# HaoruXue/spline-trajectory-optimization

Measured on AMD Instinct MI355X. Metric: min-curvature QP solves/sec (N=2000 waypoints), higher is better.
Workload: dtype f64

## Files before the change

### spline_trajectory_optimization_amd/csrc/rl_host.hpp

```cpp
#pragma once

#include "../../include/rl_mincurv.h"

#include <hip/hip_runtime.h>

#include <mutex>
#include <string>
#include <utility>
#include <vector>

namespace {

thread_local std::string g_err;

int fail(int code, const std::string& msg) {
  g_err = msg;
  return code;
}

#define RL_HIP(expr)                                                                      \
  do {                                                                                    \
    hipError_t _e = (expr);                                                               \
    if (_e != hipSuccess) {                                                               \
      return fail(RL_ERR_HIP, std::string(#expr) + ": " + hipGetErrorString(_e));         \
    }                                                                                     \
  } while (0)
#define RL_TRY(expr) do { if (int _rc = (expr)) return _rc; } while (0)

template <typename T>
struct DevBuf {
  T* p = nullptr;
  size_t n = 0;
  hipError_t alloc(size_t count) {
    release();
    n = count;
    if (count == 0) return hipSuccess;
    return hipMalloc(reinterpret_cast<void**>(&p), count * sizeof(T));
  }
  void release() {
    if (p) (void)hipFree(p);
    p = nullptr;
    n = 0;
  }
  ~DevBuf() { release(); }
  DevBuf() = default;
  DevBuf(const DevBuf&) = delete;
  DevBuf& operator=(const DevBuf&) = delete;
};

}

struct rl_ctx {
  int device = 0;
  hipStream_t stream = nullptr;
  hipEvent_t ev0 = nullptr, ev1 = nullptr;
  int max_lds = 65536;
  int num_cu = 0;
  bool force_global_v1 = false;
  int arith = RL_ARITH_REFERENCE;
  bool arith_explicit = false;
  int np_raise_at_start = 0;
  int qss_kernel = -1, qss_df_waves = 4, qss_df_bail_at = 0;
  int tables_search = RL_SEARCH_WINDOWED, tables_rings_global = 0;
  int frenet_search = 1;
  void* arena = nullptr;
  size_t arena_cap = 0;
  hipEvent_t arena_ev = nullptr;
  hipStream_t arena_stream = nullptr;
  bool arena_busy = false;
  static constexpr int kMaxGroups = 8;
  hipStream_t aux_stream[kMaxGroups - 1] = {};
  hipEvent_t ev_fork = nullptr, ev_join[kMaxGroups - 1] = {};
  hipStream_t poll_stream = nullptr;
  hipEvent_t ev_chunk[kMaxGroups] = {}, ev_poll[2] = {nullptr, nullptr};
  double* poll_host = nullptr;
  size_t poll_cap = 0;
  bool mt_hes_sweep = false;
  bool mt_kkt4 = true;
  bool mt_unfused = false;
  int mt_groups = 3;
  struct PoolBlock { void* p; size_t cap; bool used; };
  std::vector<PoolBlock> pool;
};

namespace {
hipError_t grant_dyn_lds(const rl_ctx* ctx, const void* fn, size_t bytes) {
  static std::mutex mu;
  static std::vector<std::pair<std::pair<int, const void*>, size_t>> granted;
  std::lock_guard<std::mutex> lock(mu);
  const std::pair<int, const void*> key(ctx->device, fn);
  for (auto& e : granted)
    if (e.first == key) {
      if (e.second >= bytes) return hipSuccess;
      const hipError_t r = hipFuncSetAttribute(fn, hipFuncAttributeMaxDynamicSharedMemorySize, (int)bytes);
      if (r == hipSuccess) e.second = bytes;
      return r;
    }
  const hipError_t r = hipFuncSetAttribute(fn, hipFuncAttributeMaxDynamicSharedMemorySize, (int)bytes);
  if (r == hipSuccess) granted.emplace_back(key, bytes);
  return r;
}

template <typename... P, typename... A>
int launch(const rl_ctx* ctx, hipStream_t stream, void (*kernel)(P...), dim3 grid, dim3 block, size_t lds_bytes, A&&... args) {
  if (lds_bytes > 0) RL_HIP(grant_dyn_lds(ctx, reinterpret_cast<const void*>(kernel), lds_bytes));
  hipLaunchKernelGGL(kernel, grid, block, lds_bytes, stream, static_cast<P>(std::forward<A>(args))...);
  RL_HIP(hipGetLastError());
  return RL_OK;
}
template <typename... P, typename... A>
int launch(const rl_ctx* ctx, void (*kernel)(P...), dim3 grid, dim3 block, size_t lds_bytes, A&&... args) {
  return launch(ctx, ctx->stream, kernel, grid, block, lds_bytes, std::forward<A>(args)...);
}

// ... 170 lines not shown
```

### spline_trajectory_optimization_amd/csrc/rl_mincurv.hip

```cpp
#include "rl_host.hpp"

#include <algorithm>
#include <cmath>
#include <cstdio>
#include <cstdlib>
#include <cstring>
#include <type_traits>

#include "rl_kernels.hpp"
#include "rl_sweep.hpp"
#include "rl_qss_df.hpp"
#include "rl_global.hpp"
#include "rl_global2.hpp"
#include "rl_global_xy.hpp"
#include "rl_dtrack.hpp"
#include "rl_mintime.hpp"
#include "rl_bicycle.hpp"
#include "rl_region.hpp"
#include "rl_tables.hpp"
#include "rl_pose_tables.hpp"
#include "rl_spline_fit.hpp"
#include "rl_frenet.hpp"

namespace {
// ... 264 lines not shown
    delete c;
    return fail(RL_ERR_HIP, "hipEventCreate failed");
  }
  *out = c;
  return RL_OK;
}

void rl_ctx_destroy(rl_ctx* ctx) {
  if (!ctx) return;
  if (ctx->arena) (void)hipFree(ctx->arena);
  if (ctx->arena_ev) (void)hipEventDestroy(ctx->arena_ev);
  for (auto& blk : ctx->pool)
    if (blk.p) (void)hipFree(blk.p);
  for (int g = 0; g < rl_ctx::kMaxGroups - 1; ++g) {
    if (ctx->aux_stream[g]) (void)hipStreamDestroy(ctx->aux_stream[g]);
    if (ctx->ev_join[g]) (void)hipEventDestroy(ctx->ev_join[g]);
  }
  if (ctx->ev_fork) (void)hipEventDestroy(ctx->ev_fork);
  if (ctx->poll_stream) (void)hipStreamDestroy(ctx->poll_stream);
  for (auto& e : ctx->ev_chunk) if (e) (void)hipEventDestroy(e);
  for (auto& e : ctx->ev_poll) if (e) (void)hipEventDestroy(e);
  if (ctx->poll_host) (void)hipHostFree(ctx->poll_host);
  if (ctx->ev0) (void)hipEventDestroy(ctx->ev0);
  if (ctx->ev1) (void)hipEventDestroy(ctx->ev1);
  delete ctx;
}

int rl_ctx_set_stream(rl_ctx* ctx, void* hip_stream) {
  if (!ctx) return fail(RL_ERR_ARG, "ctx is null");
  ctx->stream = reinterpret_cast<hipStream_t>(hip_stream);
  return RL_OK;
}

int rl_ctx_set_arith(rl_ctx* ctx, int arith) {
  if (!ctx) return fail(RL_ERR_ARG, "ctx is null");
  if (arith == RL_ARITH_DEFAULT) { ctx->arith = RL_ARITH_REFERENCE; ctx->arith_explicit = false; return RL_OK; }
  if (arith != RL_ARITH_FAST && arith != RL_ARITH_REFERENCE && arith != RL_ARITH_BRANCH)
    return fail(RL_ERR_ARG, "arith must be RL_ARITH_DEFAULT, RL_ARITH_FAST, RL_ARITH_REFERENCE or RL_ARITH_BRANCH");
  ctx->arith = arith;
  ctx->arith_explicit = true;
  return RL_OK;
}

int rl_ctx_get_arith(const rl_ctx* ctx) { return ctx ? (ctx->arith_explicit ? ctx->arith : RL_ARITH_DEFAULT) : RL_ERR_ARG; }

int rl_ctx_set_option(rl_ctx* ctx, const char* name, int value) {
  if (!ctx || !name) return fail(RL_ERR_ARG, "null argument");
  const std::string k(name);
  if (k == "qss_kernel") { if (value < -1 || value > 1) return fail(RL_ERR_ARG, "qss_kernel: -1 (auto), 0 (list order), 1 (dataflow)"); ctx->qss_kernel = value; }
  else if (k == "qss_df_waves") { if (value != 1 && value != 2 && value != 4) return fail(RL_ERR_ARG, "qss_df_waves: 1, 2 or 4"); ctx->qss_df_waves = value; }
  else if (k == "qss_df_bail_at") { if (value < 0) return fail(RL_ERR_ARG, "qss_df_bail_at >= 0"); ctx->qss_df_bail_at = value; }
  else if (k == "tables_search") { if (value < RL_SEARCH_BRUTE || value > RL_SEARCH_WINDOWED) return fail(RL_ERR_ARG, "tables_search: RL_SEARCH_BRUTE, _CULLED or _WINDOWED"); ctx->tables_search = value; }
  else if (k == "tables_rings") { if (value != 0 && value != 1) return fail(RL_ERR_ARG, "tables_rings: 0 (LDS where they fit) or 1 (arena)"); ctx->tables_rings_global = value; }
  else if (k == "frenet_search") { if (value != 0 && value != 1) return fail(RL_ERR_ARG, "frenet_search: 0 (table bound for every point) or 1 (from the previous point's piece)"); ctx->frenet_search = value; }
  else return fail(RL_ERR_ARG, "unknown option '" + k + "'");
  return RL_OK;
}

int rl_ctx_set_numpy_raise(rl_ctx* ctx, int on) {
  if (!ctx) return fail(RL_ERR_ARG, "ctx is null");
  ctx->np_raise_at_start = on ? 1 : 0;
  return RL_OK;
}

int rl_debug_cr_heading(rl_ctx* ctx, const double* dx, const double* dy, int n, double* out) {
  if (!ctx || !dx || !dy || !out || n <= 0) return fail(RL_ERR_ARG, "bad argument");
  Staging sg(ctx);
  const double* ddx = sg.in(dx, n);
  const double* ddy = sg.in(dy, n);
  double* dout = sg.out(out, (size_t)5 * n);
  sg.run([&] { return launch(ctx, rl::k_debug_cr_heading, dim3((n + 255) / 256), dim3(256), 0, ddx, ddy, n, dout); });
  return sg.finish();
}

int rl_ctx_synchronize(rl_ctx* ctx) {
  if (!ctx) return fail(RL_ERR_ARG, "ctx is null");
  RL_HIP(hipStreamSynchronize(ctx->stream));
  return RL_OK;
}

int rl_spline_eval(rl_ctx* ctx, const double* t, int nt, const double* cx, const double* cy, int k,
                   const double* u, int N, int der_max, double* out) {
  if (!ctx || !u || !out) return fail(RL_ERR_ARG, "null argument");
  if (int rc = check_spline(t, nt, cx, cy, k)) return rc;
  if (N <= 0 || der_max < 0 || der_max > 2) return fail(RL_ERR_ARG, "bad N / der_max");
  const int n = nt - k - 1;
  Staging sg(ctx);
  const double *dt = sg.in(t, nt), *dcx = sg.in(cx, n), *dcy = sg.in(cy, n), *du = sg.in(u, N);
  double* dout = sg.out(out, (size_t)2 * (der_max + 1) * N);
  sg.run([&] {
    return by_degree(k, [&](auto kc) {
      return launch(ctx, rl::k_spline_eval<RL_DEGREE(kc)>, dim3((N + 255) / 256), dim3(256), 0, dt, nt, dcx, dcy, du, N, der_max, dout);
    });
  });
  return sg.finish();
}

int rl_sample_along(rl_ctx* ctx, const double* t, int nt, const double* cx, const double* cy, int k,
                    double length, const double* u, int N, double* points) {
  if (!ctx || !u || !points) return fail(RL_ERR_ARG, "null argument");
  if (int rc = check_spline(t, nt, cx, cy, k)) return rc;
  if (N <= 0) return fail(RL_ERR_ARG, "bad N");
  const int n = nt - k - 1;
  Staging sg(ctx);
  const double *dt = sg.in(t, nt), *dcx = sg.in(cx, n), *dcy = sg.in(cy, n), *du = sg.in(u, N);
  double* dpts = sg.out(points, (size_t)N * RL_NCOL);
// ... 170 lines not shown
    }
    if (widest > rl::kJointRowsPerThread * 256)
      return fail(RL_ERR_UNSUPPORTED, "sliding-window variant: a window spans more than 768 samples");
  }
  int arith = ctx->arith;
  if (!ctx->arith_explicit && arith == RL_ARITH_REFERENCE && (k != 5 || (g_dbg_instances > 0 && !from))) arith = RL_ARITH_FAST;
  const bool lite = arith == RL_ARITH_BRANCH;
  const bool strict = arith == RL_ARITH_REFERENCE || lite;
  if (strict) {
    if (joint && lite) return fail(RL_ERR_UNSUPPORTED, "the branch arithmetic (rl_ctx_set_arith) covers run_min_curvature_qp; the sliding-window driver exists in the fast and in the reference-order arithmetic");
    RL_HIP(hipSetDevice(ctx->device));
    if (int rc = ensure_strict_tables(ctx, trk)) return rc;
  }
  rl::SweepArgs a;
  std::memset(&a, 0, sizeof(a));
  a.tr = trk->dev();
  a.B = B;
  a.form = form;
  a.in = in_dev;
  Bounds bd;
  if (int rc = resolve_bounds(trk, form, in_dev, bd)) return rc;
  a.ringL = bd.ringL; a.ringR = bd.ringR; a.nL = bd.nL; a.nR = bd.nR;
  a.max_iter = max_iter;
  for (int j = 0; j < max_iter && !i_start_rows; ++j) a.i_start[j] = i_start[j];
  a.ctrl0 = ctrl0; a.i_start_rows = i_start_rows;
  a.search = search;
  a.max_dist = 100.0;
#ifdef RL_ABLATION
  if (const char* dbg = getenv("RL_DEBUG_FLAGS")) a.debug = atoi(dbg);
#endif
#ifdef RL_STAMPS
  const bool dbg_ok = true;
#else
  const bool dbg_ok = !strict;
#endif
  if (g_dbg_instances > 0 && (joint || k == 5) && dbg_ok && !from) {
    const int ninst = std::min(g_dbg_instances, B);
    size_t need = joint ? (size_t)max_iter * (size_t)(i_max - i_min) * (48 + 9 * rl::kJointRowsPerThread * 256 + 2 * n)
                        : (size_t)ninst * max_iter * 2 * (size_t)(i_max - i_min) * (rl::kSweepDumpHead + 2 * n);
#ifdef RL_STAMPS
    need = std::max(need, (size_t)B * 4 * 16);
#endif
    a.dbg_instances = ninst;
    if (g_dbg_len < need) {
      if (g_dbg_buf) (void)hipFree(g_dbg_buf);
      RL_HIP(hipMalloc(reinterpret_cast<void**>(&g_dbg_buf), need * sizeof(double)));
      g_dbg_len = need;
    }
    RL_HIP(hipMemsetAsync(g_dbg_buf, 0, need * sizeof(double), ctx->stream));
    a.dbg = g_dbg_buf;
  }
  a.out_ctrl = out_ctrl; a.out_xy = out_xy; a.out_points = out_points;
  a.n_success = n_success; a.status = status;
  RL_HIP(hipSetDevice(ctx->device));
  SweepPlan p = plan_sweep(ctx, n, N, a.nL, a.nR, B, joint, strict);
  if (p.lds_bytes > (size_t)ctx->max_lds) return fail(RL_ERR_UNSUPPORTED, "problem does not fit LDS");
  if (p.residency == rl::Residency::CrossingsLds && (joint || k != 5 || a.dbg || from)) {
    p.residency = rl::Residency::Global;
    p.lds_bytes = rl::sweep_lds_layout(n, N, a.nL, a.nR, rl::Residency::Global, joint).total * sizeof(double);
    p.gscratch_doubles += (size_t)2 * ((N + 1) & ~1);
  }
  if (p.gscratch_doubles) {
    const size_t need = p.gscratch_doubles * (size_t)B;
    if (trk->gscratch.n < need) RL_HIP(trk->gscratch.alloc(need));
    a.gscratch = trk->gscratch.p;
    a.gscratch_stride = p.gscratch_doubles;
  }
  if (strict && !lite) {
    const size_t per = (size_t)2 * ((n + 1) & ~1) + (size_t)2 * ((N + 15) / 16) + (size_t)2 * N;
    const size_t flags = ((size_t)B + 1) / 2;
    if (trk->aux.n < per * (size_t)B + flags) RL_HIP(trk->aux.alloc(per * (size_t)B + flags));
    a.aux = trk->aux.p;
    a.aux_stride = per;
    a.np_raise_at_start = ctx->np_raise_at_start;
    a.raise_flag = reinterpret_cast<int*>(trk->aux.p + per * (size_t)B);
    RL_HIP(hipMemsetAsync(a.raise_flag, 0, (size_t)B * sizeof(int), ctx->stream));
  }
  if (stats) {
    stats->lds_bytes = (int)p.lds_bytes;
    stats->block_threads = p.block;
    stats->rings_in_lds = p.residency == rl::Residency::Lds ? 1 : (p.residency == rl::Residency::CrossingsLds ? 2 : 0);
    stats->reserved[0] = arith;
  }
  if (plan_out) *plan_out = p;
  if (from) return launch_sweep_from(ctx, k, p, a, strict, lite);
  return launch_sweep(ctx, k, p, a, joint, strict, lite);
}

int rl_mincurv_solve_batch_dev(rl_ctx* ctx, const rl_track* trk, int bounds_form, const double* in,
                               int B, const int* i_start, int max_iter, int search,
                               double* out_ctrl, double* out_xy, int* n_success, int* status,
                               rl_stats* stats) {
  if (!out_xy) return fail(RL_ERR_ARG, "out_xy is null");
  return solve_batch_common(ctx, trk, bounds_form, in, B, i_start, max_iter, search, out_ctrl, out_xy,
                            nullptr, n_success, status, stats, nullptr);
}

int rl_mincurv_solve_batch_host(rl_ctx* ctx, const rl_track* trk, int bounds_form, const double* in,
                                int B, const int* i_start, int max_iter, int search,
                                double* out_ctrl, double* out_xy, int* n_success, int* status,
                                rl_stats* stats) {
  if (!ctx || !trk || !out_ctrl || !out_xy) return fail(RL_ERR_ARG, "null argument");
  if (B <= 0) return fail(RL_ERR_ARG, "B <= 0");
  const int n = trk->n, N = trk->N;
  const int cols = bounds_cols(bounds_form);
  if (cols && !in) return fail(RL_ERR_ARG, "bounds input is null");
// ... 1088 lines not shown
```

### spline_trajectory_optimization_amd/csrc/rl_sweep.hpp

```cpp
#pragma once
#include "rl_kernels.hpp"

namespace rl {

constexpr int kJointRowsPerThread = 3;

struct SweepArgs {
  TrackDev tr;
  int B;
  int form;
  const double* in;
  const double2* ringL;
  const double2* ringR;
  int nL, nR;
  int max_iter;
  int i_start[32];
  int search;
  double max_dist;
  double* out_ctrl;
  double* out_xy;
  double* out_points;
  int* n_success;
  int* status;
  double* gscratch;
  size_t gscratch_stride;
  double* dbg;
  int dbg_instances;
  int debug;
  int np_raise_at_start;
  double* aux;
  size_t aux_stride;
  int* n_raised;
  int* raise_flag;
  const double* ctrl0;
  const int* i_start_rows;
};

#ifdef RL_STAMPS
#define RL_STAMP(var) do { __builtin_amdgcn_sched_barrier(0); asm volatile("s_memtime %0\n\ts_waitcnt lgkmcnt(0)" : "=s"(var) :: "memory"); __builtin_amdgcn_sched_barrier(0); } while (0)
#define RL_STAMP_ADD(slot, t1, t0) st_acc[slot] += (t1) - (t0)
#define RL_STRICT_COUNTS st_cnt
#define RL_FSTAMP(slot) do { RL_STAMP(sf1); st_fine[slot] += sf1 - sf0; sf0 = sf1; } while (0)
#else
#define RL_STAMP(var) do { } while (0)
#define RL_STAMP_ADD(slot, t1, t0) do { } while (0)
#define RL_STRICT_COUNTS nullptr
#define RL_FSTAMP(slot) do { } while (0)
#endif

#ifdef RL_ABLATION
#define RL_ABLATE(a, bit) (((a).debug & (bit)) != 0)
#else
#define RL_ABLATE(a, bit) false
#endif

enum class Residency { Lds, Global, CrossingsLds };

struct SweepLds {
  int cpad, nLp, nRp, ncL, ncR;
  size_t off_cx, off_cy, off_red, off_sL, off_sR, off_rL, off_rR, off_cL, off_cR, off_pL, off_pR, off_hint, off_joint, off_stage,
         off_c12, off_terms, total;
};
constexpr int kSweepWaves = 4;
constexpr int kSweepThreads = kWave * kSweepWaves;
constexpr int kTermChunk = 256;
constexpr int kTermStride = kTermChunk + 2;
constexpr int kC12Doubles = 4 * (2 * kMaxK) + 8;
constexpr int kRedCoordMax = 194;

__host__ __device__ inline SweepLds sweep_lds_layout(int n, int N, int nL, int nR, Residency residency,
                                                     bool joint = false, bool strict = false) {
  const bool rings_in_lds = residency == Residency::Lds, sigma_in_lds = residency != Residency::Global;
  SweepLds L;
  L.cpad = (n + 1) & ~1;
  L.nLp = nL; L.nRp = nR;
  L.ncL = (nL + kChunk - 1) / kChunk;
  L.ncR = (nR + kChunk - 1) / kChunk;
  size_t o = 0;
  L.off_cx = o; o += L.cpad;
  L.off_cy = o; o += L.cpad;
  L.off_red = o; o += 8 * 24 + 4;
  L.off_cL = o; o += (size_t)((3 * L.ncL + 1) & ~1);
  L.off_cR = o; o += (size_t)((3 * L.ncR + 1) & ~1);
  L.off_pL = o; o += (size_t)((L.ncL + 1) & ~1);
  L.off_pR = o; o += (size_t)((L.ncR + 1) & ~1);
  L.off_joint = o; o += joint ? 128 + (size_t)((N + 15) / 16) * 2 : 0;
  L.off_hint = o; o += (size_t)(((size_t)2 * ((N + 3) & ~3) * sizeof(unsigned short) + 15) / 16) * 2;
  L.off_c12 = o; o += strict ? (joint ? (size_t)4 * L.cpad : kC12Doubles) : 0;
// ... 167 lines not shown
        for (int q = 0; q < nc; ++q) {
          int dq = q - cc;
          if (dq < 0) dq = -dq;
          if (nc - dq < dq) dq = nc - dq;
          if (dq <= kNear) continue;
          const double ex = circ[3 * q] - mx, ey = circ[3 * q + 1] - my;
          gap = fmin(gap, sqrt(ex * ex + ey * ey) - r - circ[3 * q + 2]);
        }
        (left ? sepL : sepR)[cc] = gap * (1.0 - 1e-9) - 1e-9;
      }
      if (wave == 0) {
        double m = 0.0;
        for (int c = lane; c < L.ncL + L.ncR; c += kWave) {
          const double* o = c < L.ncL ? circL + 3 * c : circR + 3 * (c - L.ncL);
          const double v = fmax(fabs(o[0]), fabs(o[1])) + o[2];
          m = v <= 0x1p+1000 ? fmax(m, v) : INFINITY;
        }
        m = wave_max_bfly(m);
        if (lane == 0) red[kRedCoordMax] = m;
      }
      __syncthreads();
    }
  }

  double* jq = smem + L.off_joint;
  unsigned char* outside = reinterpret_cast<unsigned char*>(jq + 128);
  int* n_outside = reinterpret_cast<int*>(jq + 127);
  auto note_outside = [&](int i, double px, double py, double ndx, double ndy, double sl, double sr) {
    const double Lx = px + sl * ndx, Ly = py + sl * ndy;
    const double Rx = px + sr * (-ndx), Ry = py + sr * (-ndy);
    const bool out = fmin(Lx, Rx) > px || fmax(Lx, Rx) < px || fmin(Ly, Ry) > py || fmax(Ly, Ry) < py;
    const int was = outside[i];
    if ((int)out != was) { outside[i] = out ? 1 : 0; atomicAdd(n_outside, out ? 1 : -1); }
  };
  auto note_outside_pts = [&](int i, double px, double py, double2 Lp, double2 Rp) {
    const bool out = fmin(Lp.x, Rp.x) > px || fmax(Lp.x, Rp.x) < px || fmin(Lp.y, Rp.y) > py || fmax(Lp.y, Rp.y) < py;
    const int was = outside[i];
    if ((int)out != was) { outside[i] = out ? 1 : 0; atomicAdd(n_outside, out ? 1 : -1); }
  };
  if (JOINT) {
    for (int i = tid; i < N; i += BLOCK) outside[i] = 0;
    if (tid == 0) *n_outside = 0;
    __syncthreads();
  }

#ifdef RL_STAMPS
  unsigned long long st_cnt[4] = {0, 0, 0, 0};
  unsigned long long st_fine[8] = {0, 0, 0, 0, 0, 0, 0, 0}, sf0 = 0, sf1 = 0;
#endif
  unsigned char* degen = (RAISE && a.aux) ? reinterpret_cast<unsigned char*>(a.aux + (size_t)b * a.aux_stride + 2 * L.cpad) : nullptr;
  int* n_degen = reinterpret_cast<int*>(red + 190);
  bool flag_mode = false;
  bool saw_degenerate = false;
  auto refresh = [&](int i0, int i1, int j0, int j1, int mode, int l_first = -1) {
    const int m0 = i1 - i0, m1 = j1 - j0, m = m0 + m1;
    const double* cmax = red + kRedCoordMax;
    if constexpr (STRICT) {
      int delta = 0;
      auto point = [&](int i, double& px, double& py, cr::Heading& hd, bool flags, auto&& in_heading) {
#pragma clang fp contract(off)
        const int l = tr.ell[i];
        double t0[K + 1], t1[K + 1];
        load_rows<K + 1>(t0, Ds + (size_t)SR::D0 * N, N, i);
        load_rows<K + 1>(t1, Ds + (size_t)SR::D1 * N, N, i);
        __builtin_amdgcn_sched_barrier(0);
        px = seq_dot_v<K + 1>(cx + (l - K), t0);
        py = seq_dot_v<K + 1>(cy + (l - K), t0);
        const double tx = seq_dot_v<K + 1>(cx + (l - K), t1);
        const double ty = seq_dot_v<K + 1>(cy + (l - K), t1);

        if constexpr (LITE && RL_LITE_NORMAL) {
          double nx, ny, inv_s2;
          scaled_normal(tx, ty, 1.0, nx, ny, inv_s2);
          hd.cl = nx; hd.sl = ny; hd.cr = -nx; hd.sr = -ny; hd.yaw = 0.0;
          return;
        }
        if (flags) {
          const double d2x = seq_dot<K + 1>(cx + (l - K), Ds + (size_t)SR::D2 * N, N, i);
          const double d2y = seq_dot<K + 1>(cy + (l - K), Ds + (size_t)SR::D2 * N, N, i);
          const double s2 = tx * tx + ty * ty;
          const double cross = fabs(tx * d2y - ty * d2x);
          const bool plainly_regular = cross >= 0x1p-200 && cross <= 0x1p+200 && s2 >= 0x1p-100 && s2 <= 0x1p+100;
          int now = 0;
          if (!__all(plainly_regular)) {
            const double den = sqrt(s2 * s2 * s2);
            const double curvature = cross / den;
            now = (den == 0.0 || !(curvature > 0.0) || !isfinite(curvature)) ? 1 : 0;
          }
          if constexpr (RAISE) { delta += now - (int)degen[i]; degen[i] = (unsigned char)now; }
          else if (now) saw_degenerate = true;
        }
#ifdef RL_STAMPS
        unsigned long long sh0, sh1;
        RL_STAMP(sh0);
#endif
        const bool sure = cr::heading_fast(tx, ty, hd, cr::kAtanTab, nullptr, in_heading);
        if (__any(!sure)) { if (!sure) hd = cr::heading(tx, ty); }
#ifdef RL_STAMPS
        RL_STAMP(sh1); st_fine[5] += sh1 - sh0; if (__any(!sure)) st_fine[6] += 1;
#endif
      };
      if (mode == 2) {
        const int nwt = (m + kWave - 1) / kWave;
        for (int wt = wave; wt < nwt; wt += NW) {
          const int r = wt * kWave + lane;
          const bool active = r < m;
          const int i = active ? (r < m0 ? i0 + r : j0 + (r - m0)) : (m0 > 0 ? i0 : j0);
          double px, py; cr::Heading hd;
#ifdef RL_STAMPS
          RL_STAMP(sf0);
#endif
          int baseL = -1, baseR = -1;
          point(i, px, py, hd, flag_mode && active, [&]() {
            if constexpr (STAGED) {
              baseL = stage_prefetch(reinterpret_cast<const double2*>(rL), nL, L.ncL, active, (int)hints[i], stgL, lane);
              baseR = stage_prefetch(reinterpret_cast<const double2*>(rR), nR, L.ncR, active, (int)hints[Npad + i], stgR, lane);
            }
          });
          RL_FSTAMP(0);
          const double dLx = a.max_dist * hd.cl, dLy = a.max_dist * hd.sl;
          const double dRx = a.max_dist * hd.cr, dRy = a.max_dist * hd.sr;
          const Hit hl = search_ring_windowed<STAGED, true>(rL, nL, circL, sepL, L.ncL, active, (int)hints[i], px, py,
                                                            dLx, dLy, a.max_dist, cmax, false, RL_STRICT_COUNTS, stgL, baseL);
          RL_FSTAMP(1);
          const Hit hr = search_ring_windowed<STAGED, true>(rR, nR, circR, sepR, L.ncR, active, (int)hints[Npad + i], px, py,
                                                            dRx, dRy, a.max_dist, cmax, false, RL_STRICT_COUNTS, stgR, baseR);
          RL_FSTAMP(2);
          if (active) {
            const double2 Lp = make_double2(uf_madd(px, hl.best_s, dLx), uf_madd(py, hl.best_s, dLy));
            const double2 Rp = make_double2(uf_madd(px, hr.best_s, dRx), uf_madd(py, hr.best_s, dRy));
            bL[i] = Lp; bR[i] = Rp;
            hints[i] = (unsigned short)(hl.edge == kNoEdge ? 0xFFFF : hl.edge);
            hints[Npad + i] = (unsigned short)(hr.edge == kNoEdge ? 0xFFFF : hr.edge);
            if (JOINT) note_outside_pts(i, px, py, Lp, Rp);
          }
        }
        if constexpr (RAISE) { if (delta != 0) atomicAdd(n_degen, delta); }
        return;
      }
      for (int task = tid; task < 2 * m; task += BLOCK) {
        const int side = task >= m;
        const int r = side ? task - m : task;
        const int i = r < m0 ? i0 + r : j0 + (r - m0);
        double px, py; cr::Heading hd;
        point(i, px, py, hd, flag_mode && side == 0, []() {});
        const double dx = a.max_dist * (side ? hd.cr : hd.cl), dy = a.max_dist * (side ? hd.sr : hd.sl);
        Hit h;
        if (mode == 1) {
          h = side ? search_ring_culled<true>(rR, nR, circR, L.ncR, px, py, dx, dy, a.max_dist)
                   : search_ring_culled<true>(rL, nL, circL, L.ncL, px, py, dx, dy, a.max_dist);
        } else {
          h = side ? search_ring_brute<true>(rR, nR, px, py, dx, dy) : search_ring_brute<true>(rL, nL, px, py, dx, dy);
        }
        (side ? bR : bL)[i] = make_double2(uf_madd(px, h.best_s, dx), uf_madd(py, h.best_s, dy));
        hints[side * Npad + i] = (unsigned short)(h.edge == kNoEdge ? 0xFFFF : h.edge);
      }
      if constexpr (RAISE) { if (delta != 0) atomicAdd(n_degen, delta); }
      if (JOINT) {
        __syncthreads();
        for (int r = tid; r < m; r += BLOCK) {
// ... 136 lines not shown
    };
    auto knot_diffs = [&](int idx, double& d1, double& d2, double& r1, double& r2) {
      const int q = (lane + opaque_zero()) & 31;
      const int j = idx - K + q;
      d1 = 1.0; d2 = 1.0;
      if (q < 2 * K && j >= 0 && j + 1 <= n - 1) d1 = tr.t[j + K + 1] - tr.t[j + 1];
      if (q < 2 * K - 1 && j >= 0 && j + 2 <= n - 1) d2 = tr.t[j + K + 1] - tr.t[j + 2];
      r1 = rcp_chain(d1); r2 = rcp_chain(d2);
    };
    auto deriv_window = [&](int idx, double d1, double d2, double r1, double r2) {
      const int lz = lane + opaque_zero();
      const int q = lz & 31;
      const double* cc = lz < 32 ? cx : cy;
      const int j = idx - K + q;
      const bool has1 = q < 2 * K && j >= 0 && j + 1 <= n - 1, has2 = q < 2 * K - 1 && j >= 0 && j + 2 <= n - 1;
      double n1 = 0.0;
      if (has1) {
#pragma clang fp contract(off)
        n1 = (cc[j + 1] - cc[j]) * (double)K;
      }
      const bool dplain = plain_operand(d1) && d1 > 0.0 && plain_operand(d2) && d2 > 0.0;
      double c1 = 0.0, c2 = 0.0;
      if (__all(dplain && (n1 == 0.0 || plain_operand(n1)))) {
        if (has1) c1 = n1 == 0.0 ? n1 : quotient_by_chain(n1, d1, r1);
      } else {
        if (has1) c1 = n1 / d1;
      }
      const double c1n = dpp_mov<0x101, 0xf>(0.0, c1);
      double n2 = 0.0;
      if (has2) {
#pragma clang fp contract(off)
        n2 = (c1n - c1) * (double)(K - 1);
      }
      if (__all(dplain && (n2 == 0.0 || plain_operand(n2)))) {
        if (has2) c2 = n2 == 0.0 ? n2 : quotient_by_chain(n2, d2, r2);
      } else {
        if (has2) c2 = n2 / d2;
      }
      if (q < 2 * K) { c12[(lz < 32 ? 0 : 2 * K) + q] = c1; c12[4 * K + (lz < 32 ? 0 : 2 * K) + q] = c2; }
    };
    double kd1 = 1.0, kd2 = 1.0, kr1 = 1.0, kr2 = 1.0;
    if constexpr (!(LITE && RL_LITE_COST)) { if (wave == 0 && total_steps > 0) { knot_diffs(step_index(0), kd1, kd2, kr1, kr2); deriv_window(step_index(0), kd1, kd2, kr1, kr2); } }
    double2* ptab = (RAISE && a.aux) ? reinterpret_cast<double2*>(a.aux + (size_t)b * a.aux_stride + 2 * L.cpad) + ((N + 15) / 16) : nullptr;
    bool np_raise = false, stale = false;
    int raised_count = 0;
    auto sample_degenerate = [&](int i) {
#pragma clang fp contract(off)
      const int l = tr.ell[i];
      const double dx = seq_dot<K + 1>(cx + (l - K), Ds + (size_t)SR::D1 * N, N, i);
      const double dy = seq_dot<K + 1>(cy + (l - K), Ds + (size_t)SR::D1 * N, N, i);
      const double d2x = seq_dot<K + 1>(cx + (l - K), Ds + (size_t)SR::D2 * N, N, i);
      const double d2y = seq_dot<K + 1>(cy + (l - K), Ds + (size_t)SR::D2 * N, N, i);
      const double s2 = dx * dx + dy * dy;
      const double den = sqrt(s2 * s2 * s2);
      const double curvature = fabs(dx * d2y - dy * d2x) / den;
      return den == 0.0 || !(curvature > 0.0) || !isfinite(curvature);
    };
    auto flags_pass = [&](int i0, int i1, int j0, int j1) {
      const int m0 = i1 - i0, m = m0 + (j1 - j0);
      int delta = 0;
      for (int r = tid; r < m; r += BLOCK) {
        const int i = r < m0 ? i0 + r : j0 + (r - m0);
        const int now = sample_degenerate(i) ? 1 : 0;
        if constexpr (RAISE) { delta += now - (int)degen[i]; degen[i] = (unsigned char)now; }
        else if (now) saw_degenerate = true;
      }
      if constexpr (RAISE) { if (delta != 0) atomicAdd(n_degen, delta); }
    };
    __syncthreads();
    int ok_count = 0;
    auto phase1 = [&](int idx, int idx_next, int s0, int s1, double zx, double zy, double& sacc,
                      double& lox, double& hix, double& loy, double& hiy, bool& bad) {
      if constexpr (LITE && RL_LITE_COST) {
        const double* __restrict__ D2f = tr.D + (size_t)2 * (K + 1) * N;
        double hxx = 0.0, hyy = 0.0, gx = 0.0, gy = 0.0;
        for (int i = s0 + tid; i < s1; i += BLOCK) {
          const int l = tr.ell[i];
          const int aa = idx - l + K;
          {
            CurvePoint<K, 2> c;
            eval_sample<K, 2>(tr, cx, cy, i, l, c);
            const double B2 = D2f[(size_t)aa * N + i];
            double ndx, ndy, inv_s2;
            scaled_normal(c.dx, c.dy, a.max_dist, ndx, ndy, inv_s2);
            const double inv_den = inv_s2 * inv_s2 * inv_s2;
            const double Fx = c.d2x - B2 * zx, Fy = c.d2y - B2 * zy;
            const double Pxx = c.dy * c.dy * inv_den, Pyy = c.dx * c.dx * inv_den;
            const double Pxy = -2.0 * c.dx * c.dy * inv_den;
            hxx += B2 * Pxx * B2;
            hyy += B2 * Pyy * B2;
            gx += Fx * Pxx * B2;
            gy += (Fy * Pxy * B2 + Fy * Pyy * B2) + (B2 * Pxy * Fx + Fy * Pyy * B2);
          }
          {
#pragma clang fp contract(off)
            const double x = seq_dot<K + 1>(cx + (l - K), Ds + (size_t)SR::D0 * N, N, i);
            const double y = seq_dot<K + 1>(cy + (l - K), Ds + (size_t)SR::D0 * N, N, i);
            const double B0 = Ds[(size_t)(SR::D0 + aa) * N + i];
            const double2 Lp = bL[i], Rp = bR[i];
            const double nzx = x - B0 * zx, nzy = y - B0 * zy;
            const double lbx = fmin(Lp.x, Rp.x) - nzx, ubx = fmax(Lp.x, Rp.x) - nzx;
            const double lby = fmin(Lp.y, Rp.y) - nzy, uby = fmax(Lp.y, Rp.y) - nzy;
            if (B0 > 0.0) {
              lox = fmax(lox, lbx / B0); hix = fmin(hix, ubx / B0);
              loy = fmax(loy, lby / B0); hiy = fmin(hiy, uby / B0);
            } else {
              if (lbx > 0.0 || ubx < 0.0 || lby > 0.0 || uby < 0.0) bad = true;
            }
            if (!(lbx == lbx) || !(ubx == ubx) || !(lby == lby) || !(uby == uby)) bad = true;
          }
        }
        const double v0 = wave_sum(hxx), v1 = wave_sum(hyy), v2 = wave_sum(gx), v3 = wave_sum(gy);
        const double v4 = wave_max_bfly(lox), v5 = wave_min_bfly(hix), v6 = wave_max_bfly(loy), v7 = wave_min_bfly(hiy);
        const bool wbad = __any(bad);
        if (lane == 0) {
          double* r = red + wave * 12;
          r[0] = v0; r[1] = v1; r[2] = v2; r[3] = v3; r[4] = v4; r[5] = v5; r[6] = v6; r[7] = v7; r[8] = wbad ? 1.0 : 0.0;
        }
        __syncthreads();
        (void)sacc;
        return;
      }
      const int M = s1 - s0;
// ... 134 lines not shown
      double lox = -INFINITY, hix = INFINITY, loy = -INFINITY, hiy = INFINITY;
      bool bad = false;
      double sacc = 0.0;
      RL_STAMP(st_t0);
      phase1(idx, q + 1 < total_steps ? idx_n : -1, s0, s1, zx, zy, sacc, lox, hix, loy, hiy, bad);
      if (wave == 0) {
        auto lane_val = [&](int src) {
          return __hiloint2double(__builtin_amdgcn_readlane(__double2hiint(sacc), src),
                                  __builtin_amdgcn_readlane(__double2loint(sacc), src));
        };
        double t0 = lane_val(0), t1 = lane_val(1), t2 = lane_val(2), t3 = lane_val(3), t4 = lane_val(4), t5 = lane_val(5);
        if constexpr (LITE && RL_LITE_COST) {
          t0 = (red[0] + red[12]) + (red[24] + red[36]); t1 = (red[1] + red[13]) + (red[25] + red[37]);
          t2 = (red[2] + red[14]) + (red[26] + red[38]); t3 = (red[3] + red[15]) + (red[27] + red[39]);
          t4 = 0.0; t5 = 0.0;
        }
        constexpr int W0 = (LITE && RL_LITE_COST) ? 0 : 1;
        double s4 = red[W0 * 12 + 4], s5 = red[W0 * 12 + 5], s6 = red[W0 * 12 + 6], s7 = red[W0 * 12 + 7], s8 = red[W0 * 12 + 8];
        for (int w = W0 + 1; w < NW; ++w) {
          s4 = fmax(s4, red[w * 12 + 4]); s5 = fmin(s5, red[w * 12 + 5]);
          s6 = fmax(s6, red[w * 12 + 6]); s7 = fmin(s7, red[w * 12 + 7]);
          s8 = fmax(s8, red[w * 12 + 8]);
        }
        const double H0 = 2.0 * t0, H1 = 2.0 * t1;
        const double g0 = t2 + t2, g1 = (LITE && RL_LITE_COST) ? t3 : (t3 + t4) + (t5 + t4);
        const bool okw = (s8 == 0.0) && (H0 > 0.0) && (H1 > 0.0) && isfinite(H0) && isfinite(H1) &&
                         isfinite(g0) && isfinite(g1) && (s4 <= s5) && (s6 <= s7);
        if (okw) {
          double nzx = -g0 / H0, nzy = -g1 / H1;
          nzx = fmin(fmax(nzx, s4), s5);
          nzy = fmin(fmax(nzy, s6), s7);
          const int lz = lane + opaque_zero();
          if (lz < 10) {
            const bool isy = lz >= 5;
            const int c = isy ? lz - 5 : lz;
            const int src = c < 2 ? n - 5 + c : c, dst = c < 2 ? c : n - 5 + c;
            double* cc = isy ? cy : cx;
            cc[dst] = src == idx ? (isy ? nzy : nzx) : cc[src];
          } else if (lz < 12) {
            (lz == 10 ? cx : cy)[idx] = lz == 10 ? nzx : nzy;
          }
        }
        if (tid == 0) red[NW * 12] = okw ? 1.0 : 0.0;
        __builtin_amdgcn_fence(__ATOMIC_RELEASE, "workgroup");
        __builtin_amdgcn_wave_barrier();
        __builtin_amdgcn_fence(__ATOMIC_ACQUIRE, "workgroup");
        if constexpr (!(LITE && RL_LITE_COST)) { if (q + 1 < total_steps) deriv_window(idx_n, kd1, kd2, kr1, kr2); }
      }
      RL_STAMP(st_t1); RL_STAMP_ADD(2, st_t1, st_t0);
      if (wave == 0) __builtin_amdgcn_s_setprio(0);
      __syncthreads();
      RL_STAMP(st_t0); RL_STAMP_ADD(3, st_t0, st_t1);
      const bool ok = red[NW * 12] != 0.0;
      if (ok) {
        int alias = -1;
        if (idx <= 4 && idx >= 2) alias = idx + (n - 5);
        else if (idx >= n - 5 && idx <= n - 4) alias = idx - (n - 5);
        int j0 = 0, j1 = 0;
        if (alias >= 0) { j0 = tr.sup[2 * alias]; j1 = tr.sup[2 * alias + 1]; }
        const int r0 = K != 5 ? 0 : s0, r1 = K != 5 ? N : s1, q0 = K != 5 ? 0 : j0, q1 = K != 5 ? 0 : j1;
        auto write_ctrl = [&](double vx, double vy) {
          cx[idx] = vx;          cy[idx] = vy;
          cx[0] = cx[n - 5];     cy[0] = cy[n - 5];
          cx[1] = cx[n - 4];     cy[1] = cy[n - 4];
          cx[n - 3] = cx[2];     cy[n - 3] = cy[2];
          cx[n - 2] = cx[3];     cy[n - 2] = cy[3];
          cx[n - 1] = cx[4];     cy[n - 1] = cy[4];
        };
        bool raised = false;
        if constexpr (!RAISE) {
          refresh(r0, r1, q0, q1, mode);
          RL_STAMP(st_t1); RL_STAMP_ADD(4, st_t1, st_t0);
          if constexpr (RINGS_LDS || (LITE && RL_LITE_COST)) __syncthreads(); else lds_barrier();
          RL_STAMP(st_t0); RL_STAMP_ADD(5, st_t0, st_t1);
        } else {
        enum { A_NONE, A_REFRESH, A_FULL, A_UNDO };
        int act = A_REFRESH;
        if (stale) {
          flags_pass(r0, r1, q0, q1);
          __syncthreads();
          raised = *n_degen > 0;
          act = raised ? A_NONE : A_FULL;
        }
        double nzx_ = 0.0, nzy_ = 0.0;
        for (int round = 0; round < 2 && act != A_NONE; ++round) {
          const bool full = act == A_FULL;
          refresh(full ? 0 : r0, full ? N : r1, full ? 0 : q0, full ? 0 : q1, mode);
          __syncthreads();
          if (act == A_UNDO) {
            if (tid == 0) write_ctrl(nzx_, nzy_);
            flag_mode = true;
            stale = true;
            __syncthreads();
            act = A_NONE;
          } else if (act == A_FULL) {
            stale = false;
            act = A_NONE;
          } else {
            raised = np_raise && *n_degen > 0;
            act = A_NONE;
            if (raised) {
              nzx_ = cx[idx]; nzy_ = cy[idx];
              __syncthreads();
              if (tid == 0) write_ctrl(zx, zy);
              __syncthreads();
              for (int i = tid; i < N; i += BLOCK) {
                const int l = tr.ell[i];
                ptab[i] = make_double2(seq_dot<K + 1>(cx + (l - K), Ds + (size_t)SR::D0 * N, N, i),
                                       seq_dot<K + 1>(cy + (l - K), Ds + (size_t)SR::D0 * N, N, i));
              }
              flag_mode = false;
              act = A_UNDO;
            }
          }
        }
        }
        if (raised) { ++raised_count; ++n_skipped; } else ++ok_count;
      } else {
        ++n_skipped;
      }
      if (q + 1 == total_steps || stp_n == 0) {
        if (tid == 0 && a.n_success) a.n_success[(size_t)b * 2 * a.max_iter + 2 * it + pass] = ok_count;
        ok_count = 0;
      }
    }
    if (tid == 0 && a.n_raised) a.n_raised[b] = raised_count;
    if constexpr (!RAISE) { if (saw_degenerate && a.raise_flag) a.raise_flag[b] = 1; }
  } else
// ... 749 lines not shown
```

Before: 102,400.

## Defer out-of-window sweep refreshes via a range plan; add uniform regularity fast-exit

Adds an opt-in sweep_defer option that tracks pending refresh ranges in a small plan, so each accepted step re-samples only what the next step reads, padded to a 64-sample tile, and leaves the rest for later steps. The refresh routine now takes up to five ranges. The default-off non-raise path also moves through the new plan/ranges code. The degeneracy check also exits early when every lane's curvature inputs are plainly in range, skipping the sqrt and divide. The deferral feature is off by default. The restructured non-raise branch and the early-exit in the flags check may still run by default.

Result: slower. 101,000 (-1.4%).

```diff
diff --git a/spline_trajectory_optimization_amd/csrc/rl_host.hpp b/spline_trajectory_optimization_amd/csrc/rl_host.hpp
--- a/spline_trajectory_optimization_amd/csrc/rl_host.hpp
+++ b/spline_trajectory_optimization_amd/csrc/rl_host.hpp
@@ -60,6 +60,7 @@
   int arith = RL_ARITH_REFERENCE;
   bool arith_explicit = false;
   int np_raise_at_start = 0;
+  int sweep_defer = 0;
   int qss_kernel = -1, qss_df_waves = 4, qss_df_bail_at = 0;
   int tables_search = RL_SEARCH_WINDOWED, tables_rings_global = 0;
   int frenet_search = 1;
diff --git a/spline_trajectory_optimization_amd/csrc/rl_mincurv.hip b/spline_trajectory_optimization_amd/csrc/rl_mincurv.hip
--- a/spline_trajectory_optimization_amd/csrc/rl_mincurv.hip
+++ b/spline_trajectory_optimization_amd/csrc/rl_mincurv.hip
@@ -340,6 +340,7 @@
   else if (k == "qss_df_bail_at") { if (value < 0) return fail(RL_ERR_ARG, "qss_df_bail_at >= 0"); ctx->qss_df_bail_at = value; }
   else if (k == "tables_search") { if (value < RL_SEARCH_BRUTE || value > RL_SEARCH_WINDOWED) return fail(RL_ERR_ARG, "tables_search: RL_SEARCH_BRUTE, _CULLED or _WINDOWED"); ctx->tables_search = value; }
   else if (k == "tables_rings") { if (value != 0 && value != 1) return fail(RL_ERR_ARG, "tables_rings: 0 (LDS where they fit) or 1 (arena)"); ctx->tables_rings_global = value; }
+  else if (k == "sweep_defer") { if (value != 0 && value != 1) return fail(RL_ERR_ARG, "sweep_defer: 0 (a step re-samples its whole support) or 1 (what the next step reads, the rest later)"); ctx->sweep_defer = value; }
   else if (k == "frenet_search") { if (value != 0 && value != 1) return fail(RL_ERR_ARG, "frenet_search: 0 (table bound for every point) or 1 (from the previous point's piece)"); ctx->frenet_search = value; }
   else return fail(RL_ERR_ARG, "unknown option '" + k + "'");
   return RL_OK;
@@ -616,6 +617,7 @@
   }
   a.out_ctrl = out_ctrl; a.out_xy = out_xy; a.out_points = out_points;
   a.n_success = n_success; a.status = status;
+  a.sweep_defer = ctx->sweep_defer;
   RL_HIP(hipSetDevice(ctx->device));
   SweepPlan p = plan_sweep(ctx, n, N, a.nL, a.nR, B, joint, strict);
   if (p.lds_bytes > (size_t)ctx->max_lds) return fail(RL_ERR_UNSUPPORTED, "problem does not fit LDS");
diff --git a/spline_trajectory_optimization_amd/csrc/rl_refresh_plan.hpp b/spline_trajectory_optimization_amd/csrc/rl_refresh_plan.hpp
--- /dev/null
+++ b/spline_trajectory_optimization_amd/csrc/rl_refresh_plan.hpp
@@ -0,0 +1,136 @@
+#pragma once
+
+#if defined(__HIPCC__)
+#define RL_PLAN_FN __host__ __device__ __forceinline__
+#else
+#define RL_PLAN_FN inline
+#endif
+
+namespace rl {
+
+constexpr int kPlanKeep = 3;
+constexpr int kPlanSlots = kPlanKeep + 2;
+constexpr int kPlanTile = 64;
+
+struct RefreshRanges {
+  int lo[kPlanSlots], hi[kPlanSlots];
+  RL_PLAN_FN int total() const {
+    int m = 0;
+#pragma unroll
+    for (int i = 0; i < kPlanSlots; ++i) m += hi[i] - lo[i];
+    return m;
+  }
+};
+
+struct RefreshPlan {
+  int lo[kPlanSlots], hi[kPlanSlots];
+
+  RL_PLAN_FN void clear() {
+#pragma unroll
+    for (int i = 0; i < kPlanSlots; ++i) { lo[i] = 0; hi[i] = 0; }
+  }
+  RL_PLAN_FN int count() const {
+    int c = 0;
+#pragma unroll
+    for (int i = 0; i < kPlanSlots; ++i) c += hi[i] > lo[i] ? 1 : 0;
+    return c;
+  }
+  RL_PLAN_FN bool place(int a, int b) {
+    bool placed = a >= b;
+#pragma unroll
+    for (int i = 0; i < kPlanSlots; ++i) {
+      const bool here = !placed && lo[i] == hi[i];
+      lo[i] = here ? a : lo[i];
+      hi[i] = here ? b : hi[i];
+      placed = placed || here;
+    }
+    return placed;
+  }
+  RL_PLAN_FN void mark(int a, int b) {
+    if (a >= b) return;
+#pragma unroll
+    for (int i = 0; i < kPlanSlots; ++i) {
+      const bool reach = hi[i] > lo[i] && lo[i] <= b && a <= hi[i];
+      a = reach && lo[i] < a ? lo[i] : a;
+      b = reach && hi[i] > b ? hi[i] : b;
+      lo[i] = reach ? 0 : lo[i];
+      hi[i] = reach ? 0 : hi[i];
+    }
+    (void)place(a, b);
+  }
+  RL_PLAN_FN void take(int next_lo, int next_hi, bool last, RefreshRanges& out) {
+    int tlo[kPlanSlots], thi[kPlanSlots];
+    int mandatory = 0;
+#pragma unroll
+    for (int i = 0; i < kPlanSlots; ++i) {
+      const int a = lo[i] > next_lo ? lo[i] : next_lo, b = hi[i] < next_hi ? hi[i] : next_hi;
+      const bool any = a < b;
+      tlo[i] = any ? a : lo[i];
+      thi[i] = any ? b : lo[i];
+      mandatory += thi[i] - tlo[i];
+    }
+    int budget = (kPlanTile - (mandatory & (kPlanTile - 1))) & (kPlanTile - 1);
+#pragma unroll
+    for (int i = 0; i < kPlanSlots; ++i) {
+      const bool has = thi[i] > tlo[i];
+      int up = hi[i] - thi[i];
+      up = has ? (up < budget ? up : budget) : 0;
+      thi[i] += up; budget -= up;
+      int dn = tlo[i] - lo[i];
+      dn = has ? (dn < budget ? dn : budget) : 0;
+      tlo[i] -= dn; budget -= dn;
+    }
+#pragma unroll
+    for (int i = 0; i < kPlanSlots; ++i) {
+      const bool other = thi[i] == tlo[i];
+      int len = hi[i] - lo[i];
+      len = other ? (len < budget ? len : budget) : 0;
+      thi[i] += len; budget -= len;
+    }
+    int xlo = 0, xhi = 0;
+    bool fits = true;
+    RefreshPlan rest;
+#pragma unroll
+    for (int i = 0; i < kPlanSlots; ++i) {
+      const bool below = tlo[i] > lo[i], above = hi[i] > thi[i];
+      rest.lo[i] = below ? lo[i] : (above ? thi[i] : 0);
+      rest.hi[i] = below ? tlo[i] : (above ? hi[i] : 0);
+      const bool both = below && above;
+      fits = fits && !(both && xhi > xlo);
+      xlo = both ? thi[i] : xlo;
+      xhi = both ? hi[i] : xhi;
+    }
+    fits = rest.place(xlo, xhi) && fits;
+    const bool all = last || !fits || rest.count() > kPlanKeep;
+#pragma unroll
+    for (int i = 0; i < kPlanSlots; ++i) {
+      out.lo[i] = all ? lo[i] : tlo[i];
+      out.hi[i] = all ? hi[i] : thi[i];
+      lo[i] = all ? 0 : rest.lo[i];
+      hi[i] = all ? 0 : rest.hi[i];
+    }
+  }
+  RL_PLAN_FN void waiting(int a, int b, int& w0, int& w1) const {
+    int x0 = b, x1 = a;
+#pragma unroll
+    for (int i = 0; i < kPlanSlots; ++i) {
+      const int p = lo[i] > a ? lo[i] : a, q = hi[i] < b ? hi[i] : b;
+      const bool any = p < q;
+      x0 = any && p < x0 ? p : x0;
+      x1 = any && q > x1 ? q : x1;
+    }
+    const bool none = x0 >= x1;
+    w0 = none ? 0 : x0;
+    w1 = none ? 0 : x1;
+  }
+};
+
+RL_PLAN_FN void plan_step(RefreshPlan& plan, bool ok, int s0, int s1, int j0, int j1, int next_lo, int next_hi, bool last,
+                          RefreshRanges& out, int& f0, int& f1, int& g0, int& g1) {
+  if (ok) { plan.mark(s0, s1); plan.mark(j0, j1); }
+  plan.take(next_lo, next_hi, last, out);
+  f0 = f1 = g0 = g1 = 0;
+  if (ok) { plan.waiting(s0, s1, f0, f1); plan.waiting(j0, j1, g0, g1); }
+}
+
+}
diff --git a/spline_trajectory_optimization_amd/csrc/rl_sweep.hpp b/spline_trajectory_optimization_amd/csrc/rl_sweep.hpp
--- a/spline_trajectory_optimization_amd/csrc/rl_sweep.hpp
+++ b/spline_trajectory_optimization_amd/csrc/rl_sweep.hpp
@@ -1,5 +1,6 @@
 #pragma once
 #include "rl_kernels.hpp"
+#include "rl_refresh_plan.hpp"
 
 namespace rl {
 
@@ -34,6 +35,7 @@
   int* raise_flag;
   const double* ctrl0;
   const int* i_start_rows;
+  int sweep_defer;
 };
 
 #ifdef RL_STAMPS
@@ -307,7 +309,9 @@
   int* n_degen = reinterpret_cast<int*>(red + 190);
   bool flag_mode = false;
   bool saw_degenerate = false;
-  auto refresh = [&](int i0, int i1, int j0, int j1, int mode, int l_first = -1) {
+  auto refresh = [&](int i0, int i1, int j0, int j1, int mode, int l_first = -1,
+                     int x0 = 0, int x1 = 0, int y0 = 0, int y1 = 0, int z0 = 0, int z1 = 0) {
+    static_assert(kPlanSlots == 5, "refresh() takes as many ranges as the plan returns");
     const int m0 = i1 - i0, m1 = j1 - j0, m = m0 + m1;
     const double* cmax = red + kRedCoordMax;
     if constexpr (STRICT) {
@@ -356,11 +360,14 @@
 #endif
       };
       if (mode == 2) {
-        const int nwt = (m + kWave - 1) / kWave;
+        const int c1 = m, c2 = c1 + (x1 - x0), c3 = c2 + (y1 - y0), mm = c3 + (z1 - z0);
+        const int b1 = j0 - m0, b2 = x0 - c1, b3 = y0 - c2, b4 = z0 - c3;
+        const int first = m0 > 0 ? i0 : (m1 > 0 ? j0 : (c2 > c1 ? x0 : (c3 > c2 ? y0 : z0)));
+        const int nwt = (mm + kWave - 1) / kWave;
         for (int wt = wave; wt < nwt; wt += NW) {
           const int r = wt * kWave + lane;
-          const bool active = r < m;
-          const int i = active ? (r < m0 ? i0 + r : j0 + (r - m0)) : (m0 > 0 ? i0 : j0);
+          const bool active = r < mm;
+          const int i = active ? r + (r < m0 ? i0 : (r < c1 ? b1 : (r < c2 ? b2 : (r < c3 ? b3 : b4)))) : first;
           double px, py; cr::Heading hd;
 #ifdef RL_STAMPS
           RL_STAMP(sf0);
@@ -603,8 +610,11 @@
       const double d2x = seq_dot<K + 1>(cx + (l - K), Ds + (size_t)SR::D2 * N, N, i);
       const double d2y = seq_dot<K + 1>(cy + (l - K), Ds + (size_t)SR::D2 * N, N, i);
       const double s2 = dx * dx + dy * dy;
+      const double cross = fabs(dx * d2y - dy * d2x);
+      const bool plainly_regular = cross >= 0x1p-200 && cross <= 0x1p+200 && s2 >= 0x1p-100 && s2 <= 0x1p+100;
+      if (__all(plainly_regular)) return false;
       const double den = sqrt(s2 * s2 * s2);
-      const double curvature = fabs(dx * d2y - dy * d2x) / den;
+      const double curvature = cross / den;
       return den == 0.0 || !(curvature > 0.0) || !isfinite(curvature);
     };
     auto flags_pass = [&](int i0, int i1, int j0, int j1) {
@@ -620,6 +630,9 @@
     };
     __syncthreads();
     int ok_count = 0;
+    RefreshPlan plan;
+    plan.clear();
+    const bool defer = !RAISE && K == 5 && mode == 2 && a.sweep_defer != 0;
     auto phase1 = [&](int idx, int idx_next, int s0, int s1, double zx, double zy, double& sacc,
                       double& lox, double& hix, double& loy, double& hiy, bool& bad) {
       if constexpr (LITE && RL_LITE_COST) {
@@ -860,6 +873,34 @@
       __syncthreads();
       RL_STAMP(st_t0); RL_STAMP_ADD(3, st_t0, st_t1);
       const bool ok = red[NW * 12] != 0.0;
+      if constexpr (!RAISE) {
+        const bool oku = __builtin_amdgcn_readfirstlane(ok ? 1 : 0) != 0;
+        int j0 = 0, j1 = 0;
+        if (oku) {
+          int alias = -1;
+          if (idx <= 4 && idx >= 2) alias = idx + (n - 5);
+          else if (idx >= n - 5 && idx <= n - 4) alias = idx - (n - 5);
+          if (alias >= 0) { j0 = tr.sup[2 * alias]; j1 = tr.sup[2 * alias + 1]; }
+        }
+        RefreshRanges rr;
+        int f0 = 0, f1 = 0, g0 = 0, g1 = 0;
+        if (defer) {
+          plan_step(plan, oku, s0, s1, j0, j1, __builtin_amdgcn_readfirstlane(s0_n), __builtin_amdgcn_readfirstlane(s1_n),
+                    q + 1 == total_steps, rr, f0, f1, g0, g1);
+        } else {
+#pragma unroll
+          for (int u = 0; u < kPlanSlots; ++u) { rr.lo[u] = 0; rr.hi[u] = 0; }
+          if (oku) { rr.lo[0] = K != 5 ? 0 : s0; rr.hi[0] = K != 5 ? N : s1; rr.lo[1] = K != 5 ? 0 : j0; rr.hi[1] = K != 5 ? 0 : j1; }
+        }
+        if (flag_mode && (f1 > f0 || g1 > g0)) flags_pass(f0, f1, g0, g1);
+        if (rr.total() > 0) {
+          refresh(rr.lo[0], rr.hi[0], rr.lo[1], rr.hi[1], mode, -1, rr.lo[2], rr.hi[2], rr.lo[3], rr.hi[3], rr.lo[4], rr.hi[4]);
+          RL_STAMP(st_t1); RL_STAMP_ADD(4, st_t1, st_t0);
+          if constexpr (RINGS_LDS || (LITE && RL_LITE_COST)) __syncthreads(); else lds_barrier();
+          RL_STAMP(st_t0); RL_STAMP_ADD(5, st_t0, st_t1);
+        }
+        if (oku) ++ok_count; else ++n_skipped;
+      } else
       if (ok) {
         int alias = -1;
         if (idx <= 4 && idx >= 2) alias = idx + (n - 5);
@@ -876,12 +917,7 @@
           cx[n - 1] = cx[4];     cy[n - 1] = cy[4];
         };
         bool raised = false;
-        if constexpr (!RAISE) {
-          refresh(r0, r1, q0, q1, mode);
-          RL_STAMP(st_t1); RL_STAMP_ADD(4, st_t1, st_t0);
-          if constexpr (RINGS_LDS || (LITE && RL_LITE_COST)) __syncthreads(); else lds_barrier();
-          RL_STAMP(st_t0); RL_STAMP_ADD(5, st_t0, st_t1);
-        } else {
+        {
         enum { A_NONE, A_REFRESH, A_FULL, A_UNDO };
         int act = A_REFRESH;
         if (stale) {
```
